# jameschapman19/cca_zoo

Hardware: NVIDIA H100
Metric: rcca_fit_per_s (higher is better)
Workload: dtype tf32x3b+f32

## Files before the change

### cca_zoo_b200/csrc/common.cuh

```cuda
#pragma once

#include <cuda.h>
#include <cuda_runtime.h>
#include <stdint.h>
#include <stdio.h>

namespace ccab {

void set_error(const char* fmt, ...);
int cuda_fail(cudaError_t e, const char* what);

#define CCAB_CUDA(expr)                                              \
  do {                                                               \
    cudaError_t _e = (expr);                                         \
    if (_e != cudaSuccess) return ::ccab::cuda_fail(_e, #expr);      \
  } while (0)

#define CCAB_CHECK_ARG(cond, ...)        \
  do {                                   \
    if (!(cond)) {                       \
      ::ccab::set_error(__VA_ARGS__);    \
      return -1;                         \
    }                                    \
  } while (0)

void count_launches(int n);
long launch_count();

static inline int64_t ceil_div(int64_t a, int64_t b) { return (a + b - 1) / b; }

#ifdef __CUDACC__

__device__ __forceinline__ uint32_t smem_u32(const void* p) {
  return static_cast<uint32_t>(__cvta_generic_to_shared(p));
}

template <int N>
__device__ __forceinline__ void setmaxnreg_dec() { asm volatile("setmaxnreg.dec.sync.aligned.u32 %0;" ::"n"(N)); }
template <int N>
__device__ __forceinline__ void setmaxnreg_inc() { asm volatile("setmaxnreg.inc.sync.aligned.u32 %0;" ::"n"(N)); }

__device__ __forceinline__ void mbar_init(uint64_t* bar, uint32_t count) {
  asm volatile("mbarrier.init.shared::cta.b64 [%0], %1;" ::"r"(smem_u32(bar)), "r"(count) : "memory");
}
__device__ __forceinline__ void fence_mbar_init() {
  asm volatile("fence.mbarrier_init.release.cluster;" ::: "memory");
}
__device__ __forceinline__ void mbar_arrive(uint64_t* bar) {
  asm volatile("mbarrier.arrive.shared::cta.b64 _, [%0];" ::"r"(smem_u32(bar)) : "memory");
}
__device__ __forceinline__ void mbar_arrive_expect_tx(uint64_t* bar, uint32_t bytes) {
  asm volatile("mbarrier.arrive.expect_tx.shared::cta.b64 _, [%0], %1;" ::"r"(smem_u32(bar)), "r"(bytes)
               : "memory");
}
__device__ __forceinline__ bool mbar_try_wait(uint64_t* bar, uint32_t parity) {
  uint32_t ok;
  asm volatile(
      "{\n\t.reg .pred P1;\n\t"
      "mbarrier.try_wait.parity.shared::cta.b64 P1, [%1], %2;\n\t"
      "selp.b32 %0, 1, 0, P1;\n\t}\n"
      : "=r"(ok)
      : "r"(smem_u32(bar)), "r"(parity)
      : "memory");
  return ok != 0;
}
__device__ __forceinline__ void mbar_wait(uint64_t* bar, uint32_t parity) {
  uint32_t spins = 0;
  while (!mbar_try_wait(bar, parity)) {
    if (++spins > (1u << 25)) __trap();
  }
}

__device__ __forceinline__ void tma_load_2d(void* smem_dst, const CUtensorMap* map, uint64_t* bar, int c0, int c1) {
  asm volatile(
      "cp.async.bulk.tensor.2d.shared::cluster.global.mbarrier::complete_tx::bytes [%0], [%1, {%3, %4}], [%2];"
      ::"r"(smem_u32(smem_dst)), "l"(map), "r"(smem_u32(bar)), "r"(c0), "r"(c1)
      : "memory");
}


__device__ __forceinline__ void fence_proxy_async_smem() {
  asm volatile("fence.proxy.async.shared::cta;" ::: "memory");
}
__device__ __forceinline__ void wgmma_fence() { asm volatile("wgmma.fence.sync.aligned;" ::: "memory"); }
__device__ __forceinline__ void wgmma_commit() { asm volatile("wgmma.commit_group.sync.aligned;" ::: "memory"); }
__device__ __forceinline__ void wgmma_wait_all() { asm volatile("wgmma.wait_group.sync.aligned 0;" ::: "memory"); }
__device__ __forceinline__ void wgmma_wait_1() { asm volatile("wgmma.wait_group.sync.aligned 1;" ::: "memory"); }
template <int R>
__device__ __forceinline__ void wgmma_fence_regs(float* d) {
#pragma unroll
  for (int i = 0; i < R; ++i) asm volatile("" : "+f"(d[i])::"memory");
}

__device__ __forceinline__ uint64_t wgmma_desc_k128(uint32_t saddr) {
  return (uint64_t)((saddr >> 4) & 0x3FFF) | ((uint64_t)1 << 16) | ((uint64_t)(1024 >> 4) << 32) |
         ((uint64_t)1 << 62);
}

template <int N>
__device__ __forceinline__ void wgmma_tf32(float* d, uint64_t desc_a, uint64_t desc_b);

template <>
__device__ __forceinline__ void wgmma_tf32<64>(float* d, uint64_t desc_a, uint64_t desc_b) {
  asm volatile(
      "{\n\t.reg .pred p;\n\tsetp.ne.b32 p, %34, 0;\n\t"
      "wgmma.mma_async.sync.aligned.m64n64k8.f32.tf32.tf32 "
      "{%0, %1, %2, %3, %4, %5, %6, %7, %8, %9, %10, %11, %12, %13, %14, %15, %16, %17, %18, %19, %20, %21, %22, %23, %24, %25, %26, %27, %28, %29, %30, %31}, %32, %33, p, 1, 1;\n\t}\n"
      : "+f"(d[0]), "+f"(d[1]), "+f"(d[2]), "+f"(d[3]), "+f"(d[4]), "+f"(d[5]), "+f"(d[6]), "+f"(d[7]), "+f"(d[8]), "+f"(d[9]), "+f"(d[10]), "+f"(d[11]), "+f"(d[12]), "+f"(d[13]), "+f"(d[14]), "+f"(d[15]), "+f"(d[16]), "+f"(d[17]), "+f"(d[18]), "+f"(d[19]), "+f"(d[20]), "+f"(d[21]), "+f"(d[22]), "+f"(d[23]), "+f"(d[24]), "+f"(d[25]), "+f"(d[26]), "+f"(d[27]), "+f"(d[28]), "+f"(d[29]), "+f"(d[30]), "+f"(d[31])
      : "l"(desc_a), "l"(desc_b), "r"(1));
}

template <>
__device__ __forceinline__ void wgmma_tf32<128>(float* d, uint64_t desc_a, uint64_t desc_b) {
  asm volatile(
      "{\n\t.reg .pred p;\n\tsetp.ne.b32 p, %66, 0;\n\t"
      "wgmma.mma_async.sync.aligned.m64n128k8.f32.tf32.tf32 "
      "{%0, %1, %2, %3, %4, %5, %6, %7, %8, %9, %10, %11, %12, %13, %14, %15, %16, %17, %18, %19, %20, %21, %22, %23, %24, %25, %26, %27, %28, %29, %30, %31, %32, %33, %34, %35, %36, %37, %38, %39, %40, %41, %42, %43, %44, %45, %46, %47, %48, %49, %50, %51, %52, %53, %54, %55, %56, %57, %58, %59, %60, %61, %62, %63}, %64, %65, p, 1, 1;\n\t}\n"
      : "+f"(d[0]), "+f"(d[1]), "+f"(d[2]), "+f"(d[3]), "+f"(d[4]), "+f"(d[5]), "+f"(d[6]), "+f"(d[7]), "+f"(d[8]), "+f"(d[9]), "+f"(d[10]), "+f"(d[11]), "+f"(d[12]), "+f"(d[13]), "+f"(d[14]), "+f"(d[15]), "+f"(d[16]), "+f"(d[17]), "+f"(d[18]), "+f"(d[19]), "+f"(d[20]), "+f"(d[21]), "+f"(d[22]), "+f"(d[23]), "+f"(d[24]), "+f"(d[25]), "+f"(d[26]), "+f"(d[27]), "+f"(d[28]), "+f"(d[29]), "+f"(d[30]), "+f"(d[31]), "+f"(d[32]), "+f"(d[33]), "+f"(d[34]), "+f"(d[35]), "+f"(d[36]), "+f"(d[37]), "+f"(d[38]), "+f"(d[39]), "+f"(d[40]), "+f"(d[41]), "+f"(d[42]), "+f"(d[43]), "+f"(d[44]), "+f"(d[45]), "+f"(d[46]), "+f"(d[47]), "+f"(d[48]), "+f"(d[49]), "+f"(d[50]), "+f"(d[51]), "+f"(d[52]), "+f"(d[53]), "+f"(d[54]), "+f"(d[55]), "+f"(d[56]), "+f"(d[57]), "+f"(d[58]), "+f"(d[59]), "+f"(d[60]), "+f"(d[61]), "+f"(d[62]), "+f"(d[63])
      : "l"(desc_a), "l"(desc_b), "r"(1));
}

__device__ __forceinline__ float tf32_hi(float v) { return __uint_as_float(__float_as_uint(v) & 0xFFFFE000u); }
__device__ __forceinline__ float tf32_residual(float v) {
  uint32_t l;
  asm("cvt.rna.tf32.f32 %0, %1;" : "=r"(l) : "f"(v - tf32_hi(v)));
  return __uint_as_float(l);
}

__device__ __forceinline__ uint32_t k128_offset(int row, int kg) {
  return (uint32_t)row * 128u + ((uint32_t)(kg ^ (row & 7)) << 4);
}

template <bool KMAJ, int ROWS>
struct TileStager {
  static constexpr int kItems = ROWS * 8 / 256;
  float v[kItems][4];

  __device__ __forceinline__ static int item_row(int i) { return KMAJ ? i >> 3 : i % ROWS; }
  __device__ __forceinline__ static int item_kg(int i) { return KMAJ ? i & 7 : i / ROWS; }

  __device__ __forceinline__ void load(const float* X, int64_t ld, int rows, int ks, bool vec) {
#pragma unroll
    for (int j = 0; j < kItems; ++j) {
      const int i = threadIdx.x + 256 * j;
      const int r = item_row(i), k = 4 * item_kg(i);
      if (KMAJ) {
        const float* src = X + (int64_t)r * ld + k;
        if (vec && r < rows && k + 4 <= ks) {
          const float4 q = __ldg(reinterpret_cast<const float4*>(src));
          v[j][0] = q.x; v[j][1] = q.y; v[j][2] = q.z; v[j][3] = q.w;
        } else {
#pragma unroll
          for (int e = 0; e < 4; ++e) v[j][e] = (r < rows && k + e < ks) ? __ldg(src + e) : 0.f;
        }
      } else {
#pragma unroll
        for (int e = 0; e < 4; ++e) v[j][e] = (r < rows && k + e < ks) ? __ldg(X + (int64_t)(k + e) * ld + r) : 0.f;
      }
    }
  }

  template <bool X3>
  __device__ __forceinline__ void store(uint8_t* hi, uint8_t* lo) const {
#pragma unroll
    for (int j = 0; j < kItems; ++j) {
      const int i = threadIdx.x + 256 * j;
      const uint32_t off = k128_offset(item_row(i), item_kg(i));
      *reinterpret_cast<float4*>(hi + off) =
          make_float4(tf32_hi(v[j][0]), tf32_hi(v[j][1]), tf32_hi(v[j][2]), tf32_hi(v[j][3]));
      if (X3)
        *reinterpret_cast<float4*>(lo + off) = make_float4(tf32_residual(v[j][0]), tf32_residual(v[j][1]),
                                                           tf32_residual(v[j][2]), tf32_residual(v[j][3]));
    }
  }
};

#endif

}
```

### cca_zoo_b200/csrc/moments.cu

```cuda
#include "moments.cuh"

#include <mutex>
#include <type_traits>

namespace ccab {

int make_layout(int n_views, const int64_t* dims, ColumnLayout* L) {
  CCAB_CHECK_ARG(n_views >= 1 && n_views <= kMaxViews, "n_views must be in [1,%d], got %d", kMaxViews,
                 n_views);
  L->n_views = n_views;
  L->coff[0] = 0;
  L->poff[0] = 0;
  int nb = 0;
  for (int v = 0; v < n_views; ++v) {
    CCAB_CHECK_ARG(dims[v] >= 1 && dims[v] <= kMaxBlocks * kBlk, "bad view width %lld", (long long)dims[v]);
    L->dims[v] = (int)dims[v];
    int b = (int)ceil_div(dims[v], kBlk);
    nb += b;
    L->coff[v + 1] = L->coff[v] + (int)dims[v];
    L->poff[v + 1] = L->poff[v] + b * kBlk;
  }
  CCAB_CHECK_ARG(nb <= kMaxBlocks, "total padded width %d exceeds %d", nb * kBlk, kMaxBlocks * kBlk);
  L->nblocks = nb;
  L->D = L->coff[n_views];
  L->Dp = nb * kBlk;
  return 0;
}

static bool g_prof_on = false;
static cudaEvent_t g_prof_e0 = nullptr, g_prof_e1 = nullptr;
static bool g_prof_valid = false;
void moments_profile_enable(int on) {
  g_prof_on = on != 0;
  g_prof_valid = false;
  if (g_prof_on && !g_prof_e0) {
    cudaEventCreate(&g_prof_e0);
    cudaEventCreate(&g_prof_e1);
  }
}
float moments_profile_last_ms() {
  if (!g_prof_valid) return -1.f;
  float ms = -1.f;
  if (cudaEventSynchronize(g_prof_e1) != cudaSuccess) return -1.f;
  if (cudaEventElapsedTime(&ms, g_prof_e0, g_prof_e1) != cudaSuccess) return -1.f;
  return ms;
}

struct WgParams {
  CUtensorMap map[kMaxViews];
  uint8_t blk_view[kMaxBlocks];
  int blk_col0[kMaxBlocks];
  float* partial;
  float* partial_sum;
  int64_t n_rows, rows_per_split;
  int64_t row_base;
  int nblocks, Dp;
};
static_assert(sizeof(WgParams) <= 4096, "kernel parameter space");

constexpr int kWgXpose = 256;
constexpr int kWgThreads = kWgXpose + 256;
constexpr int kWgKC = 32;
constexpr int kWgTile = kBlk * kWgKC * 4;

template <bool X3>
struct WgCfg {
  static constexpr int kOps = X3 ? 2 : 1;
  static constexpr int kOpStage = 2 * kOps * kWgTile;
  static constexpr int kRawStage = 2 * kWgTile;
  static constexpr int kOpStages = X3 ? 2 : 3;
  static constexpr int kRawStages = X3 ? 3 : 4;
  static constexpr int kBarOff = kOpStages * kOpStage + kRawStages * kRawStage;
  static constexpr int kSumOff = kBarOff + 2 * (kOpStages + kRawStages) * 8;
  static constexpr int kSmem = kSumOff + kBlk * 4 + 1024;
};
static_assert(WgCfg<true>::kSmem <= 227 * 1024 && WgCfg<false>::kSmem <= 227 * 1024, "shared memory per block");

template <bool X3>
__global__ void __launch_bounds__(kWgThreads, 1) moments_wgmma_kernel(const __grid_constant__ WgParams p) {
  using Cfg = WgCfg<X3>;
  constexpr int NO = Cfg::kOpStages, NR = Cfg::kRawStages;
  extern __shared__ uint8_t smem_raw[];
  uint8_t* smem = smem_raw + ((1024u - (smem_u32(smem_raw) & 1023u)) & 1023u);
  uint8_t* ops = smem;
  uint8_t* raw = smem + NO * Cfg::kOpStage;
  uint64_t* raw_full = reinterpret_cast<uint64_t*>(smem + Cfg::kBarOff);
  uint64_t* raw_empty = raw_full + NR;
  uint64_t* op_full = raw_empty + NR;
  uint64_t* op_empty = op_full + NO;

  int t = blockIdx.x, bi = 0, rowlen = p.nblocks;
  while (t >= rowlen) { t -= rowlen; ++bi; --rowlen; }
  const int bj = bi + t;
  const bool diag = bi == bj;
  const int split = blockIdx.y;
  const int64_t r0 = (int64_t)split * p.rows_per_split;
  const int64_t r1 = min(r0 + p.rows_per_split, p.n_rows);
  const int nch = r1 > r0 ? (int)((r1 - r0 + kWgKC - 1) / kWgKC) : 0;

  if (threadIdx.x == 0) {
    for (int s = 0; s < NR; ++s) {
      mbar_init(&raw_full[s], 1);
      mbar_init(&raw_empty[s], kWgXpose);
    }
    for (int s = 0; s < NO; ++s) {
      mbar_init(&op_full[s], kWgXpose);
      mbar_init(&op_empty[s], 8);
    }
    fence_mbar_init();
  }
  __syncthreads();

  if (threadIdx.x < kWgXpose) {
    setmaxnreg_dec<80>();
    const int m = threadIdx.x % kBlk, h = threadIdx.x / kBlk;
    const CUtensorMap* mapA = &p.map[p.blk_view[bi]];
    const CUtensorMap* mapB = &p.map[p.blk_view[bj]];
    const int colA = p.blk_col0[bi], colB = p.blk_col0[bj];
    auto issue = [&](int c) {
      const int s = c % NR;
      const int row = (int)(p.row_base + r0 + (int64_t)c * kWgKC);
      mbar_arrive_expect_tx(&raw_full[s], diag ? kWgTile : 2 * kWgTile);
      tma_load_2d(raw + s * Cfg::kRawStage, mapA, &raw_full[s], colA, row);
      if (!diag) tma_load_2d(raw + s * Cfg::kRawStage + kWgTile, mapB, &raw_full[s], colB, row);
    };
    if (threadIdx.x == 0)
      for (int c = 0; c < min(NR, nch); ++c) issue(c);

    float csum = 0.f;
    auto transpose = [&](const float* src, uint8_t* hi, uint8_t* lo, bool sums) {
#pragma unroll
      for (int j = 0; j < kWgKC / 8; ++j) {
        const int kg = 2 * j + h;
        float v[4];
#pragma unroll
        for (int e = 0; e < 4; ++e) v[e] = src[(4 * kg + e) * kBlk + m];
        const uint32_t off = k128_offset(m, kg);
        *reinterpret_cast<float4*>(hi + off) = make_float4(tf32_hi(v[0]), tf32_hi(v[1]), tf32_hi(v[2]), tf32_hi(v[3]));
        if (X3)
          *reinterpret_cast<float4*>(lo + off) = make_float4(tf32_residual(v[0]), tf32_residual(v[1]),
                                                             tf32_residual(v[2]), tf32_residual(v[3]));
        if (sums) csum += (v[0] + v[1]) + (v[2] + v[3]);
      }
    };
    for (int c = 0; c < nch; ++c) {
      const int sr = c % NR, so = c % NO;
      mbar_wait(&raw_full[sr], (c / NR) & 1);
      mbar_wait(&op_empty[so], ((c / NO) & 1) ^ 1);
      const float* src = reinterpret_cast<const float*>(raw + sr * Cfg::kRawStage);
      uint8_t* dst = ops + so * Cfg::kOpStage;
      transpose(src, dst, dst + kWgTile, diag);
      if (!diag) transpose(src + kBlk * kWgKC, dst + Cfg::kOps * kWgTile, dst + (Cfg::kOps + 1) * kWgTile, false);
      fence_proxy_async_smem();
      mbar_arrive(&raw_empty[sr]);
      mbar_arrive(&op_full[so]);
      if (threadIdx.x == 0 && c + NR < nch) {
        mbar_wait(&raw_empty[sr], (c / NR) & 1);
        issue(c + NR);
      }
    }
    if (diag) {
      float* odd = reinterpret_cast<float*>(smem + Cfg::kSumOff);
      if (h) odd[m] = csum;
      asm volatile("bar.sync 1, %0;" ::"n"(kWgXpose) : "memory");
      if (!h) p.partial_sum[(size_t)split * p.Dp + bi * kBlk + m] = csum + odd[m];
    }
  } else {
    setmaxnreg_inc<168>();
    const int wg = (threadIdx.x - kWgXpose) >> 7;
    float acc[64];
#pragma unroll
    for (int i = 0; i < 64; ++i) acc[i] = 0.f;
    wgmma_fence_regs<64>(acc);
    for (int c = 0; c < nch; ++c) {
      const int so = c % NO;
      mbar_wait(&op_full[so], (c / NO) & 1);
      const uint32_t st = smem_u32(ops + so * Cfg::kOpStage);
      const uint32_t a0 = st + wg * 64 * 128;
      const uint32_t b0 = diag ? st : st + Cfg::kOps * kWgTile;
      wgmma_fence();
#pragma unroll
      for (int kk = 0; kk < kWgKC / 8; ++kk) {
        const uint64_t a_hi = wgmma_desc_k128(a0 + 32 * kk), b_hi = wgmma_desc_k128(b0 + 32 * kk);
        if (X3) {
          const uint64_t a_lo = wgmma_desc_k128(a0 + kWgTile + 32 * kk), b_lo = wgmma_desc_k128(b0 + kWgTile + 32 * kk);
          wgmma_tf32<128>(acc, a_lo, b_hi);
          wgmma_tf32<128>(acc, a_hi, b_lo);
        }
        wgmma_tf32<128>(acc, a_hi, b_hi);
      }
      wgmma_commit();
      wgmma_wait_1();
      if (c > 0 && (threadIdx.x & 31) == 0) mbar_arrive(&op_empty[(c - 1) % NO]);
    }
    wgmma_wait_all();
    wgmma_fence_regs<64>(acc);

    const int warp = (threadIdx.x >> 5) & 3, lane = threadIdx.x & 31;
    float* P = p.partial + (size_t)split * p.Dp * p.Dp;
    const int row0 = bi * kBlk + wg * 64 + warp * 16 + (lane >> 2);
    const int col0 = bj * kBlk + 2 * (lane & 3);
#pragma unroll
    for (int r = 0; r < 64; r += 2) {
      const int row = row0 + 8 * ((r >> 1) & 1), col = col0 + 8 * (r >> 2);
      *reinterpret_cast<float2*>(P + (size_t)row * p.Dp + col) = make_float2(acc[r], acc[r + 1]);
    }
  }
}
struct SimtParams {
  const void* view_ptr[kMaxViews];
  int64_t view_ld[kMaxViews];
  int view_dim[kMaxViews];
  int view_poff[kMaxViews + 1];
  int n_views;
  int64_t n_rows;
  int64_t rows_per_split;
  int nb64, Dp;
  void* partial;
  void* partial_sum;
};

template <typename T>
__global__ void __launch_bounds__(256) moments_simt_kernel(const SimtParams p) {
  constexpr int KC = 16;
  __shared__ T As[KC][64];
  __shared__ T Bs[KC][64];
  int t = blockIdx.x, bi = 0, rowlen = p.nb64;
  while (t >= rowlen) { t -= rowlen; ++bi; --rowlen; }
  const int bj = bi + t;
  const int split = blockIdx.y;
  const int64_t r0 = split * p.rows_per_split;
  const int64_t r1 = min(r0 + p.rows_per_split, p.n_rows);

  auto locate = [&](int pcol0, int& v, int& c0) {
    v = 0;
    while (v + 1 < p.n_views && p.view_poff[v + 1] <= pcol0) ++v;
    c0 = pcol0 - p.view_poff[v];
  };
  int vA, cA, vB, cB;
  locate(bi * 64, vA, cA);
  locate(bj * 64, vB, cB);
  const T* XA = static_cast<const T*>(p.view_ptr[vA]);
  const T* XB = static_cast<const T*>(p.view_ptr[vB]);
  const int64_t ldA = p.view_ld[vA], ldB = p.view_ld[vB];
  const int dA = p.view_dim[vA], dB = p.view_dim[vB];

  const int tx = threadIdx.x & 15, ty = threadIdx.x >> 4;
  T acc[4][4];
#pragma unroll
  for (int i = 0; i < 4; ++i)
#pragma unroll
    for (int j = 0; j < 4; ++j) acc[i][j] = T(0);
  T csum[4] = {T(0), T(0), T(0), T(0)};

  const int lc = threadIdx.x & 63, lr = threadIdx.x >> 6;
  for (int64_t r = r0; r < r1; r += KC) {
#pragma unroll
    for (int i = 0; i < KC / 4; ++i) {
      const int kr = lr + 4 * i;
      const int64_t row = r + kr;
      const bool rv = row < r1;
      As[kr][lc] = (rv && cA + lc < dA) ? XA[row * ldA + cA + lc] : T(0);
      Bs[kr][lc] = (rv && cB + lc < dB) ? XB[row * ldB + cB + lc] : T(0);
    }
    __syncthreads();
#pragma unroll
    for (int k = 0; k < KC; ++k) {
      T a[4], b[4];
#pragma unroll
      for (int i = 0; i < 4; ++i) { a[i] = As[k][ty * 4 + i]; b[i] = Bs[k][tx * 4 + i]; }
#pragma unroll
      for (int i = 0; i < 4; ++i)
#pragma unroll
        for (int j = 0; j < 4; ++j) acc[i][j] = fma(a[i], b[j], acc[i][j]);
      if (ty == 0) {
#pragma unroll
        for (int j = 0; j < 4; ++j) csum[j] += b[j];
      }
    }
    __syncthreads();
  }
  T* P = static_cast<T*>(p.partial) + (size_t)split * p.Dp * p.Dp;
#pragma unroll
  for (int i = 0; i < 4; ++i)
#pragma unroll
    for (int j = 0; j < 4; ++j)
      P[(size_t)(bi * 64 + ty * 4 + i) * p.Dp + bj * 64 + tx * 4 + j] = acc[i][j];
  if (bi == bj && ty == 0) {
    T* S = static_cast<T*>(p.partial_sum) + (size_t)split * p.Dp;
#pragma unroll
    for (int j = 0; j < 4; ++j) S[bi * 64 + tx * 4 + j] = csum[j];
  }
}

__device__ __forceinline__ void dmma_m8n8k4(double& c0, double& c1, double a, double b) {
  asm volatile("mma.sync.aligned.m8n8k4.row.col.f64.f64.f64.f64 {%0, %1}, {%2}, {%3}, {%0, %1};"
               : "+d"(c0), "+d"(c1)
               : "d"(a), "d"(b));
}

__global__ void __launch_bounds__(256) moments_dmma_kernel(const SimtParams p) {
  constexpr int KC = 16;
  constexpr int LDS = 64 + 4;
  __shared__ double As[2][KC][LDS];
  __shared__ double Bs[2][KC][LDS];
  int t = blockIdx.x, bi = 0, rowlen = p.nb64;
  while (t >= rowlen) { t -= rowlen; ++bi; --rowlen; }
  const int bj = bi + t;
  const int split = blockIdx.y;
  const int64_t r0 = split * p.rows_per_split;
  const int64_t r1 = min(r0 + p.rows_per_split, p.n_rows);

  auto locate = [&](int pcol0, int& v, int& c0) {
    v = 0;
    while (v + 1 < p.n_views && p.view_poff[v + 1] <= pcol0) ++v;
    c0 = pcol0 - p.view_poff[v];
  };
  int vA, cA, vB, cB;
  locate(bi * 64, vA, cA);
  locate(bj * 64, vB, cB);
  const double* XA = static_cast<const double*>(p.view_ptr[vA]);
  const double* XB = static_cast<const double*>(p.view_ptr[vB]);
  const int64_t ldA = p.view_ld[vA], ldB = p.view_ld[vB];
  const int dA = p.view_dim[vA], dB = p.view_dim[vB];

  const int warp = threadIdx.x >> 5, lane = threadIdx.x & 31;
  const int wm = (warp & 1) * 32, wn = (warp >> 1) * 16;
  const int gq = lane >> 2, tq = lane & 3;
  double acc[4][2][2];
#pragma unroll
  for (int i = 0; i < 4; ++i)
#pragma unroll
    for (int j = 0; j < 2; ++j) acc[i][j][0] = acc[i][j][1] = 0.0;
  double csum = 0.0;

  const int lc = threadIdx.x & 63, lr = threadIdx.x >> 6;
  double ra[KC / 4], rb[KC / 4];
  auto gload = [&](int64_t r) {
#pragma unroll
    for (int i = 0; i < KC / 4; ++i) {
      const int64_t row = r + lr + 4 * i;
      const bool rv = row < r1;
      ra[i] = (rv && cA + lc < dA) ? XA[row * ldA + cA + lc] : 0.0;
      rb[i] = (rv && cB + lc < dB) ? XB[row * ldB + cB + lc] : 0.0;
    }
  };
  auto sstore = [&](int buf) {
#pragma unroll
    for (int i = 0; i < KC / 4; ++i) {
      As[buf][lr + 4 * i][lc] = ra[i];
      Bs[buf][lr + 4 * i][lc] = rb[i];
    }
  };
  gload(r0);
  sstore(0);
  __syncthreads();
  int buf = 0;
  for (int64_t r = r0; r < r1; r += KC, buf ^= 1) {
    const bool more = r + KC < r1;
    if (more) gload(r + KC);
#pragma unroll
    for (int k0 = 0; k0 < KC; k0 += 4) {
      double a[4], b[2];
#pragma unroll
      for (int i = 0; i < 4; ++i) a[i] = As[buf][k0 + tq][wm + 8 * i + gq];
#pragma unroll
      for (int j = 0; j < 2; ++j) b[j] = Bs[buf][k0 + tq][wn + 8 * j + gq];
#pragma unroll
      for (int i = 0; i < 4; ++i)
#pragma unroll
        for (int j = 0; j < 2; ++j) dmma_m8n8k4(acc[i][j][0], acc[i][j][1], a[i], b[j]);
    }
    if (bi == bj && threadIdx.x < 64) {
#pragma unroll
      for (int k = 0; k < KC; ++k) csum += Bs[buf][k][threadIdx.x];
    }
    if (more) sstore(buf ^ 1);
    __syncthreads();
  }
  double* P = static_cast<double*>(p.partial) + (size_t)split * p.Dp * p.Dp;
#pragma unroll
  for (int i = 0; i < 4; ++i)
#pragma unroll
    for (int j = 0; j < 2; ++j) {
      const int row = bi * 64 + wm + 8 * i + gq;
      const int col = bj * 64 + wn + 8 * j + 2 * tq;
      *reinterpret_cast<double2*>(P + (size_t)row * p.Dp + col) = make_double2(acc[i][j][0], acc[i][j][1]);
    }
  if (bi == bj && threadIdx.x < 64)
    static_cast<double*>(p.partial_sum)[(size_t)split * p.Dp + bi * 64 + threadIdx.x] = csum;
}

template <typename T>
__global__ void reduce_partials_kernel(const T* __restrict__ partial, const T* __restrict__ partial_sum,
                                       int S, int Dp, int ldp, int blk, double* __restrict__ out,
                                       int accumulate = 0) {
  const size_t total = (size_t)Dp * Dp + (partial_sum ? Dp : 0);
  const size_t slab = (size_t)ldp * ldp;
  for (size_t i = blockIdx.x * (size_t)blockDim.x + threadIdx.x; i < total;
       i += (size_t)gridDim.x * blockDim.x) {
    double acc = 0.0;
    if (i < (size_t)Dp * Dp) {
      const int r = (int)(i / Dp), c = (int)(i % Dp);
      if (r / blk <= c / blk) {
        const T* src = partial + (size_t)r * ldp + c;
        int s = 0;
        for (; s + 8 <= S; s += 8) {
          T v[8];
#pragma unroll
          for (int u = 0; u < 8; ++u) v[u] = src[(size_t)(s + u) * slab];
#pragma unroll
          for (int u = 0; u < 8; ++u) acc += (double)v[u];
        }
        for (; s < S; ++s) acc += (double)src[(size_t)s * slab];
      }
    } else {
      const size_t j = i - (size_t)Dp * Dp;
      for (int s = 0; s < S; ++s) acc += (double)partial_sum[(size_t)s * ldp + j];
    }
    out[i] = accumulate ? out[i] + acc : acc;
  }
}

struct CovParams {
  int n_views, D, Dp;
  int dims[kMaxViews];
  int coff[kMaxViews + 1];
  int poff[kMaxViews + 1];
};

__device__ __forceinline__ int compact_to_padded(const CovParams& p, int g) {
  int v = 0;
  while (v + 1 < p.n_views && p.coff[v + 1] <= g) ++v;
  return p.poff[v] + (g - p.coff[v]);
}

template <typename Tout>
__global__ void covariance_kernel(const CovParams p, const double* __restrict__ mom, double n_total,
                                  int center, Tout* __restrict__ C, int64_t ldc, Tout* __restrict__ mean) {
  const double* M = mom;
  const double* s = mom + (size_t)p.Dp * p.Dp;
  const int gi = blockIdx.y * blockDim.y + threadIdx.y;
  const int gj = blockIdx.x * blockDim.x + threadIdx.x;
  if (gi >= p.D || gj >= p.D) return;
  const int pi = compact_to_padded(p, gi), pj = compact_to_padded(p, gj);
  const int r = min(pi, pj), c = max(pi, pj);
  double v = M[(size_t)r * p.Dp + c];
  if (center) v -= s[pi] * s[pj] / n_total;
  C[(size_t)gi * ldc + gj] = (Tout)(v / (n_total - 1.0));
  if (gi == 0 && mean) mean[gj] = (Tout)(center ? s[pj] / n_total : 0.0);
}

namespace {

int sm_count() {
  static int n[64] = {};
  int dev = 0;
  cudaGetDevice(&dev);
  if (dev < 0 || dev >= 64) return 132;
  if (!n[dev]) {
    cudaDeviceGetAttribute(&n[dev], cudaDevAttrMultiProcessorCount, dev);
    if (n[dev] <= 0) n[dev] = 132;
  }
  return n[dev];
}

struct TcPlan {
  int total_chunks, num_splits, chunks_per_split, ntiles;
  size_t partial_bytes, sum_bytes;
};

TcPlan plan_tc(const ColumnLayout& L, int64_t n_rows, int mode) {
  const bool x3 = mode != 0;
  TcPlan P;
  P.total_chunks = (int)ceil_div(n_rows, kWgKC);
  P.ntiles = L.nblocks * (L.nblocks + 1) / 2;
  int S = (int)ceil_div(4 * sm_count(), P.ntiles);
  int max_splits = 64;
  if (x3) {
    S = std::max<int64_t>(S, ceil_div(n_rows, 2048));
    max_splits = 256;
  }
  const int min_chunks = 8;
  S = (int)std::min<int64_t>(S, std::max<int64_t>(1, P.total_chunks / min_chunks));
  const int64_t slab = (int64_t)L.Dp * L.Dp * (int64_t)sizeof(float);
  max_splits = (int)std::max<int64_t>(1, std::min<int64_t>(max_splits, ((int64_t)2 << 30) / slab));
  S = std::min(S, max_splits);
  S = std::max(1, std::min(S, P.total_chunks));
  P.chunks_per_split = (int)ceil_div(P.total_chunks, S);
  P.num_splits = (int)ceil_div(P.total_chunks, P.chunks_per_split);
  P.partial_bytes = (size_t)P.num_splits * L.Dp * L.Dp * sizeof(float);
  P.sum_bytes = (size_t)P.num_splits * L.Dp * sizeof(float);
  return P;
}

int64_t tc_rows_cap(const ColumnLayout& L, int mode) {
  if (mode == 0) return (int64_t)1 << 31;
  const int64_t slab = (int64_t)L.Dp * L.Dp * (int64_t)sizeof(float);
  const int64_t max_splits = std::max<int64_t>(1, std::min<int64_t>(256, ((int64_t)2 << 30) / slab));
  return max_splits * 2048;
}

inline size_t align256(size_t x) { return (x + 255) & ~size_t(255); }

struct SimtPlan {
  int nb64, ntiles, num_splits;
  int64_t rows_per_split;
};

SimtPlan plan_simt(const ColumnLayout& L, int64_t n_rows) {
  SimtPlan P;
  P.nb64 = L.Dp / 64;
  P.ntiles = P.nb64 * (P.nb64 + 1) / 2;
  int S = 1;
  if (P.ntiles < 2 * sm_count()) S = (2 * sm_count()) / P.ntiles;
  S = (int)std::min<int64_t>(S, std::max<int64_t>(1, n_rows / 64));
  S = std::max(1, std::min(S, 64));
  P.rows_per_split = ceil_div(ceil_div(n_rows, S), 16) * 16;
  P.num_splits = (int)ceil_div(n_rows, P.rows_per_split);
  return P;
}

}

size_t moments_workspace_bytes(int dtype, int precision, const ColumnLayout& L, int64_t n_rows) {
  if (precision == 2 || dtype == 1) {
    SimtPlan P = plan_simt(L, n_rows);
    size_t el = dtype == 1 ? 8 : 4;
    return align256((size_t)P.num_splits * L.Dp * L.Dp * el) + align256((size_t)P.num_splits * L.Dp * el);
  }
  TcPlan P = plan_tc(L, std::min(n_rows, tc_rows_cap(L, precision)), precision);
  return align256(P.partial_bytes) + align256(P.sum_bytes) + 256;
}

namespace {

typedef CUresult (*EncodeTiledFn)(CUtensorMap*, CUtensorMapDataType, cuuint32_t, void*, const cuuint64_t*,
                                  const cuuint64_t*, const cuuint32_t*, const cuuint32_t*, CUtensorMapInterleave,
                                  CUtensorMapSwizzle, CUtensorMapL2promotion, CUtensorMapFloatOOBfill);

EncodeTiledFn encode_fn() {
  static EncodeTiledFn fn = nullptr;
  static std::once_flag once;
  std::call_once(once, [] {
    void* f = nullptr;
    cudaDriverEntryPointQueryResult q;
    if (cudaGetDriverEntryPoint("cuTensorMapEncodeTiled", &f, cudaEnableDefault, &q) == cudaSuccess &&
        q == cudaDriverEntryPointSuccess)
      fn = reinterpret_cast<EncodeTiledFn>(f);
  });
  return fn;
}

int encode_view_map(CUtensorMap* map, const void* ptr, int64_t n_rows, int64_t d, int64_t ld) {
  EncodeTiledFn enc = encode_fn();
  if (!enc) {
    set_error("cuTensorMapEncodeTiled entry point not available (driver too old?)");
    return -2;
  }
  cuuint64_t gdim[2] = {(cuuint64_t)d, (cuuint64_t)n_rows};
  cuuint64_t gstride[1] = {(cuuint64_t)ld * 4};
  cuuint32_t box[2] = {(cuuint32_t)kBlk, (cuuint32_t)kWgKC};
  cuuint32_t estr[2] = {1, 1};
  CUresult r = enc(map, CU_TENSOR_MAP_DATA_TYPE_FLOAT32, 2, const_cast<void*>(ptr), gdim, gstride, box, estr,
                   CU_TENSOR_MAP_INTERLEAVE_NONE, CU_TENSOR_MAP_SWIZZLE_NONE, CU_TENSOR_MAP_L2_PROMOTION_L2_256B,
                   CU_TENSOR_MAP_FLOAT_OOB_FILL_NONE);
  if (r != CUDA_SUCCESS) {
    set_error("cuTensorMapEncodeTiled failed with CUresult %d (d=%lld n=%lld ld=%lld)", (int)r, (long long)d,
              (long long)n_rows, (long long)ld);
    return -3;
  }
  return 0;
}

int moments_tf32_pass(const ColumnLayout& L, WgParams& prm, int64_t row_base, int64_t n_rows, int mode,
                      double* moments_out, void* ws, size_t ws_bytes, cudaStream_t stream, int accumulate);

}

int moments_tf32(const ColumnLayout& L, const void* const* views, const int64_t* lds, int64_t n_rows, int mode,
                 double* moments_out, void* ws, size_t ws_bytes, cudaStream_t stream) {
  CCAB_CHECK_ARG(n_rows >= 1 && n_rows < (int64_t)1 << 31, "n_rows out of range");
  for (int v = 0; v < L.n_views; ++v)
    CCAB_CHECK_ARG((reinterpret_cast<uintptr_t>(views[v]) & 15) == 0 && lds[v] % 4 == 0,
                   "TF32 moments need 16-byte aligned views and lds %% 4 == 0 (view %d: ld %lld)", v,
                   (long long)lds[v]);
  {
    int dev = 0;
    CCAB_CUDA(cudaGetDevice(&dev));
    CCAB_CUDA(cudaSetDevice(dev));
  }
  WgParams prm;
  memset(&prm, 0, sizeof(prm));
  for (int v = 0; v < L.n_views; ++v) {
    int rc = encode_view_map(&prm.map[v], views[v], n_rows, L.dims[v], lds[v]);
    if (rc) return rc;
  }
  int b = 0;
  for (int v = 0; v < L.n_views; ++v)
    for (int c = 0; c < L.dims[v]; c += kBlk, ++b) {
      prm.blk_view[b] = (uint8_t)v;
      prm.blk_col0[b] = c;
    }
  const int64_t cap = tc_rows_cap(L, mode);
  if (n_rows <= cap) return moments_tf32_pass(L, prm, 0, n_rows, mode, moments_out, ws, ws_bytes, stream, 0);
  const int64_t npass = ceil_div(n_rows, cap);
  const int64_t per = std::min(cap, ceil_div(ceil_div(n_rows, npass), 2048) * 2048);
  int pass = 0;
  for (int64_t r0 = 0; r0 < n_rows; r0 += per, ++pass) {
    int rc = moments_tf32_pass(L, prm, r0, std::min(per, n_rows - r0), mode, moments_out, ws, ws_bytes, stream,
                               pass > 0);
    if (rc) return rc;
  }
  return 0;
}

namespace {
int moments_tf32_pass(const ColumnLayout& L, WgParams& prm, int64_t row_base, int64_t n_rows, int mode,
                      double* moments_out, void* ws, size_t ws_bytes, cudaStream_t stream, int accumulate) {
  TcPlan P = plan_tc(L, n_rows, mode);
  const size_t need = align256(P.partial_bytes) + align256(P.sum_bytes) + 256;
  CCAB_CHECK_ARG(ws_bytes >= need, "workspace too small: %zu < %zu", ws_bytes, need);
  uint8_t* w = reinterpret_cast<uint8_t*>((reinterpret_cast<uintptr_t>(ws) + 255) & ~uintptr_t(255));
  float* d_partial = reinterpret_cast<float*>(w);
  float* d_partial_sum = reinterpret_cast<float*>(w + align256(P.partial_bytes));

  prm.partial = d_partial;
  prm.partial_sum = d_partial_sum;
  prm.n_rows = n_rows;
  prm.rows_per_split = (int64_t)P.chunks_per_split * kWgKC;
  prm.row_base = row_base;
  prm.nblocks = L.nblocks;
  prm.Dp = L.Dp;
  dim3 grid(P.ntiles, P.num_splits);
  if (g_prof_on) cudaEventRecord(g_prof_e0, stream);
  if (mode != 0) {
    CCAB_CUDA(cudaFuncSetAttribute(moments_wgmma_kernel<true>, cudaFuncAttributeMaxDynamicSharedMemorySize,
                                   WgCfg<true>::kSmem));
    moments_wgmma_kernel<true><<<grid, kWgThreads, WgCfg<true>::kSmem, stream>>>(prm);
  } else {
    CCAB_CUDA(cudaFuncSetAttribute(moments_wgmma_kernel<false>, cudaFuncAttributeMaxDynamicSharedMemorySize,
                                   WgCfg<false>::kSmem));
    moments_wgmma_kernel<false><<<grid, kWgThreads, WgCfg<false>::kSmem, stream>>>(prm);
  }
  count_launches(1);
  CCAB_CUDA(cudaGetLastError());
  if (g_prof_on) {
    cudaEventRecord(g_prof_e1, stream);
    g_prof_valid = true;
  }

  const size_t total = (size_t)L.Dp * L.Dp + L.Dp;
  int rblocks = (int)std::min<size_t>((total + 255) / 256, (size_t)sm_count() * 8);
  reduce_partials_kernel<float><<<rblocks, 256, 0, stream>>>(d_partial, d_partial_sum, P.num_splits, L.Dp, L.Dp,
                                                            kBlk, moments_out, accumulate); count_launches(1);
  CCAB_CUDA(cudaGetLastError());
  return 0;
}
}

template <typename T>
int moments_simt(const ColumnLayout& L, const void* const* views, const int64_t* lds, int64_t n_rows,
                 double* moments_out, void* ws, size_t ws_bytes, cudaStream_t stream) {
  CCAB_CHECK_ARG(n_rows >= 1, "n_rows must be positive");
  SimtPlan P = plan_simt(L, n_rows);
  const size_t pb = align256((size_t)P.num_splits * L.Dp * L.Dp * sizeof(T));
  const size_t sb = align256((size_t)P.num_splits * L.Dp * sizeof(T));
  CCAB_CHECK_ARG(ws_bytes >= pb + sb, "workspace too small: %zu < %zu", ws_bytes, pb + sb);
  uint8_t* w = static_cast<uint8_t*>(ws);
  SimtParams prm;
  memset(&prm, 0, sizeof(prm));
  for (int v = 0; v < L.n_views; ++v) {
    prm.view_ptr[v] = views[v];
    prm.view_ld[v] = lds[v];
    prm.view_dim[v] = L.dims[v];
  }
  for (int v = 0; v <= L.n_views; ++v) prm.view_poff[v] = L.poff[v];
  prm.n_views = L.n_views;
  prm.n_rows = n_rows;
  prm.rows_per_split = P.rows_per_split;
  prm.nb64 = P.nb64;
  prm.Dp = L.Dp;
  prm.partial = w;
  prm.partial_sum = w + pb;
  dim3 grid(P.ntiles, P.num_splits);
  if constexpr (std::is_same<T, double>::value)
    moments_dmma_kernel<<<grid, 256, 0, stream>>>(prm);
  else
    moments_simt_kernel<T><<<grid, 256, 0, stream>>>(prm);
  count_launches(1);
  CCAB_CUDA(cudaGetLastError());
  const size_t total = (size_t)L.Dp * L.Dp + L.Dp;
  int rblocks = (int)std::min<size_t>((total + 255) / 256, (size_t)sm_count() * 8);
  reduce_partials_kernel<T><<<rblocks, 256, 0, stream>>>(static_cast<const T*>(prm.partial),
                                                        static_cast<const T*>(prm.partial_sum), P.num_splits,
                                                        L.Dp, L.Dp, 64, moments_out); count_launches(1);
  CCAB_CUDA(cudaGetLastError());
  return 0;
}

template int moments_simt<float>(const ColumnLayout&, const void* const*, const int64_t*, int64_t, double*, void*,
                                 size_t, cudaStream_t);
template int moments_simt<double>(const ColumnLayout&, const void* const*, const int64_t*, int64_t, double*, void*,
                                  size_t, cudaStream_t);

__global__ void pack_moments_kernel(const double* __restrict__ mom, int nblocks, int Dp, double n_local,
                                    double* __restrict__ packed) {
  const int nt = nblocks * (nblocks + 1) / 2;
  const int t = blockIdx.x;
  if (t < nt) {
    int bi = 0, rem = t, rowlen = nblocks;
    while (rem >= rowlen) { rem -= rowlen; ++bi; --rowlen; }
    const int bj = bi + rem;
    const double* src = mom + (size_t)bi * kBlk * Dp + (size_t)bj * kBlk;
    double* dst = packed + (size_t)t * kBlk * kBlk;
    for (int e = threadIdx.x; e < kBlk * kBlk; e += blockDim.x) dst[e] = src[(size_t)(e / kBlk) * Dp + (e % kBlk)];
  } else {
    double* dst = packed + (size_t)nt * kBlk * kBlk;
    const double* s = mom + (size_t)Dp * Dp;
    for (int e = threadIdx.x; e < Dp; e += blockDim.x) dst[e] = s[e];
    if (threadIdx.x == 0) { dst[Dp] = n_local; dst[Dp + 1] = 0.0; }
  }
}

__global__ void unpack_moments_kernel(const double* __restrict__ packed, int nblocks, int Dp, double* __restrict__ mom) {
  const int nt = nblocks * (nblocks + 1) / 2;
  const int bi = blockIdx.y, bj = blockIdx.x;
  if (bi < nblocks) {
    double* dst = mom + (size_t)bi * kBlk * Dp + (size_t)bj * kBlk;
    if (bj >= bi) {
      const int t = bi * nblocks - bi * (bi - 1) / 2 + (bj - bi);
      const double* src = packed + (size_t)t * kBlk * kBlk;
      for (int e = threadIdx.x; e < kBlk * kBlk; e += blockDim.x) dst[(size_t)(e / kBlk) * Dp + (e % kBlk)] = src[e];
    } else {
      for (int e = threadIdx.x; e < kBlk * kBlk; e += blockDim.x) dst[(size_t)(e / kBlk) * Dp + (e % kBlk)] = 0.0;
    }
  } else if (bj == 0) {
    const double* src = packed + (size_t)nt * kBlk * kBlk;
    double* s = mom + (size_t)Dp * Dp;
    for (int e = threadIdx.x; e < Dp; e += blockDim.x) s[e] = src[e];
  }
}

__device__ __forceinline__ double multimem_ld_reduce_add_f64(const double* mc_addr) {
  double v;
  asm volatile("multimem.ld_reduce.relaxed.sys.global.add.f64 %0, [%1];" : "=d"(v) : "l"(mc_addr) : "memory");
  return v;
}
__device__ __forceinline__ void multimem_st_f64(double* mc_addr, double v) {
  asm volatile("multimem.st.relaxed.sys.global.f64 [%0], %1;" ::"l"(mc_addr), "d"(v) : "memory");
}
__device__ __forceinline__ void st_release_sys_u32(uint32_t* p, uint32_t v) {
  asm volatile("st.release.sys.global.u32 [%0], %1;" ::"l"(p), "r"(v) : "memory");
}
__device__ __forceinline__ uint32_t ld_acquire_sys_u32(const uint32_t* p) {
  uint32_t v;
  asm volatile("ld.acquire.sys.global.u32 %0, [%1];" : "=r"(v) : "l"(p) : "memory");
  return v;
}

struct ExchangeParams {
  double* mom;
  double* sym;
  double* mc;
  uint32_t* const* pads;
  double* n_total_out;
  double n_local;
  long long packed;
  long long chunk;
  int rank, world, nblocks, Dp;
  unsigned epoch;
};

__device__ __forceinline__ const double* packed_src(const ExchangeParams& p, long long e, int nt) {
  const long long blk = e / (kBlk * kBlk);
  if (blk < nt) {
    int bi = 0, rem = (int)blk, rowlen = p.nblocks;
    while (rem >= rowlen) { rem -= rowlen; ++bi; --rowlen; }
    const int bj = bi + rem;
    const int off = (int)(e - blk * (kBlk * kBlk));
    return p.mom + ((size_t)bi * kBlk + off / kBlk) * p.Dp + (size_t)bj * kBlk + (off % kBlk);
  }
  const long long t = e - (long long)nt * kBlk * kBlk;
  return t < p.Dp ? p.mom + (size_t)p.Dp * p.Dp + t : nullptr;
}

__device__ __forceinline__ void exchange_barrier(const ExchangeParams& p, unsigned value) {
  __threadfence_system();
  __syncthreads();
  if ((int)threadIdx.x < p.world)
    st_release_sys_u32(p.pads[threadIdx.x] + (size_t)blockIdx.x * p.world + p.rank, value);
  if ((int)threadIdx.x < p.world) {
    const uint32_t* slot = p.pads[p.rank] + (size_t)blockIdx.x * p.world + threadIdx.x;
    unsigned spins = 0;
    while ((int)(ld_acquire_sys_u32(slot) - value) < 0) {
      if (++spins > (1u << 26)) {
        printf("ccab: exchange barrier timed out (rank %d cta %d peer %d)\n", p.rank, blockIdx.x, threadIdx.x);
        __trap();
      }
    }
  }
  __syncthreads();
}

__global__ void __launch_bounds__(512) exchange_nvls_kernel(const ExchangeParams p) {
  const int nt = p.nblocks * (p.nblocks + 1) / 2;
  const long long sub = (p.chunk + gridDim.x - 1) / gridDim.x;
  const long long r0 = (long long)blockIdx.x * sub;
  const long long r1 = r0 + sub < p.chunk ? r0 + sub : p.chunk;
  for (int rho = 0; rho < p.world; ++rho) {
    const long long base = (long long)rho * p.chunk;
    for (long long i = r0 + threadIdx.x; i < r1; i += blockDim.x) {
      const long long e = base + i;
      double v = 0.0;
      if (e < p.packed) {
        const double* src = packed_src(p, e, nt);
        v = src ? *src : (e == (long long)nt * kBlk * kBlk + p.Dp ? p.n_local : 0.0);
      }
      p.sym[e] = v;
    }
  }
  exchange_barrier(p, p.epoch);
  {
    const long long base = (long long)p.rank * p.chunk;
    for (long long i = r0 + threadIdx.x; i < r1; i += blockDim.x) {
      const double v = multimem_ld_reduce_add_f64(p.mc + base + i);
      multimem_st_f64(p.mc + base + i, v);
    }
  }
  exchange_barrier(p, p.epoch + 1);
  for (int rho = 0; rho < p.world; ++rho) {
    const long long base = (long long)rho * p.chunk;
    for (long long i = r0 + threadIdx.x; i < r1; i += blockDim.x) {
      const long long e = base + i;
      if (e >= p.packed) continue;
      const double v = p.sym[e];
      const double* dst = packed_src(p, e, nt);
      if (dst) *const_cast<double*>(dst) = v;
      else if (e == (long long)nt * kBlk * kBlk + p.Dp && p.n_total_out) *p.n_total_out = v;
    }
  }
}

int moments_exchange_nvls(const ColumnLayout& L, double* mom, double n_local, double* sym_local, double* sym_multicast,
                          void* const* pads_dev, int rank, int world, int pad_slots, int64_t sym_doubles,
                          unsigned epoch, double* n_total_out, cudaStream_t stream) {
  CCAB_CHECK_ARG(world >= 2 && world <= 64 && rank >= 0 && rank < world, "bad rank / world %d / %d", rank, world);
  CCAB_CHECK_ARG(mom && sym_local && sym_multicast && pads_dev, "null pointer argument");
  ExchangeParams p;
  memset(&p, 0, sizeof(p));
  p.mom = mom; p.sym = sym_local; p.mc = sym_multicast;
  p.pads = reinterpret_cast<uint32_t* const*>(pads_dev);
  p.n_total_out = n_total_out; p.n_local = n_local;
  p.packed = moments_packed_size(L);
  p.chunk = ceil_div(ceil_div(p.packed, world), 2) * 2;
  CCAB_CHECK_ARG(sym_doubles >= p.chunk * world, "symmetric buffer too small: %lld < %lld doubles", (long long)sym_doubles,
                 (long long)(p.chunk * world));
  p.rank = rank; p.world = world; p.nblocks = L.nblocks; p.Dp = L.Dp; p.epoch = epoch;
  int grid = std::min(64, pad_slots / world);
  CCAB_CHECK_ARG(grid >= 1, "signal pad too small for %d ranks", world);
  grid = (int)std::min<int64_t>(grid, std::max<int64_t>(1, p.chunk / 512));
  exchange_nvls_kernel<<<grid, 512, 0, stream>>>(p);
  count_launches(1);
  CCAB_CUDA(cudaGetLastError());
  return 0;
}

template <typename T>
// ... 157 lines not shown
```

Measured before the change: 115.6.

## Feed wgmma A operand from registers loaded directly from swizzled raw TMA tiles

The MMA warpgroups now read the A-side tile straight from the raw TMA stage into registers, split it into tf32 hi/lo parts there, and issue register-A wgmma. The transpose warps only produce the B-side operand tile, which halves the op stage size. TMA loads switch to 32-column boxes with 128B swizzle so the register reads avoid bank conflicts. Raw stages go up to five, and the refill schedule and barrier counts change so the MMA warps also release raw stages. In exchange, the MMA warps do more scalar work, use more registers, and the barrier protocol becomes more intricate.

```diff
diff --git a/cca_zoo_b200/csrc/common.cuh b/cca_zoo_b200/csrc/common.cuh
--- a/cca_zoo_b200/csrc/common.cuh
+++ b/cca_zoo_b200/csrc/common.cuh
@@ -86,10 +86,17 @@
 __device__ __forceinline__ void wgmma_commit() { asm volatile("wgmma.commit_group.sync.aligned;" ::: "memory"); }
 __device__ __forceinline__ void wgmma_wait_all() { asm volatile("wgmma.wait_group.sync.aligned 0;" ::: "memory"); }
 __device__ __forceinline__ void wgmma_wait_1() { asm volatile("wgmma.wait_group.sync.aligned 1;" ::: "memory"); }
+template <int N>
+__device__ __forceinline__ void wgmma_wait() { asm volatile("wgmma.wait_group.sync.aligned %0;" ::"n"(N) : "memory"); }
 template <int R>
 __device__ __forceinline__ void wgmma_fence_regs(float* d) {
 #pragma unroll
   for (int i = 0; i < R; ++i) asm volatile("" : "+f"(d[i])::"memory");
+}
+template <int R>
+__device__ __forceinline__ void wgmma_fence_regs(uint32_t* a) {
+#pragma unroll
+  for (int i = 0; i < R; ++i) asm volatile("" : "+r"(a[i])::"memory");
 }
 
 __device__ __forceinline__ uint64_t wgmma_desc_k128(uint32_t saddr) {
@@ -118,6 +125,19 @@
       "{%0, %1, %2, %3, %4, %5, %6, %7, %8, %9, %10, %11, %12, %13, %14, %15, %16, %17, %18, %19, %20, %21, %22, %23, %24, %25, %26, %27, %28, %29, %30, %31, %32, %33, %34, %35, %36, %37, %38, %39, %40, %41, %42, %43, %44, %45, %46, %47, %48, %49, %50, %51, %52, %53, %54, %55, %56, %57, %58, %59, %60, %61, %62, %63}, %64, %65, p, 1, 1;\n\t}\n"
       : "+f"(d[0]), "+f"(d[1]), "+f"(d[2]), "+f"(d[3]), "+f"(d[4]), "+f"(d[5]), "+f"(d[6]), "+f"(d[7]), "+f"(d[8]), "+f"(d[9]), "+f"(d[10]), "+f"(d[11]), "+f"(d[12]), "+f"(d[13]), "+f"(d[14]), "+f"(d[15]), "+f"(d[16]), "+f"(d[17]), "+f"(d[18]), "+f"(d[19]), "+f"(d[20]), "+f"(d[21]), "+f"(d[22]), "+f"(d[23]), "+f"(d[24]), "+f"(d[25]), "+f"(d[26]), "+f"(d[27]), "+f"(d[28]), "+f"(d[29]), "+f"(d[30]), "+f"(d[31]), "+f"(d[32]), "+f"(d[33]), "+f"(d[34]), "+f"(d[35]), "+f"(d[36]), "+f"(d[37]), "+f"(d[38]), "+f"(d[39]), "+f"(d[40]), "+f"(d[41]), "+f"(d[42]), "+f"(d[43]), "+f"(d[44]), "+f"(d[45]), "+f"(d[46]), "+f"(d[47]), "+f"(d[48]), "+f"(d[49]), "+f"(d[50]), "+f"(d[51]), "+f"(d[52]), "+f"(d[53]), "+f"(d[54]), "+f"(d[55]), "+f"(d[56]), "+f"(d[57]), "+f"(d[58]), "+f"(d[59]), "+f"(d[60]), "+f"(d[61]), "+f"(d[62]), "+f"(d[63])
       : "l"(desc_a), "l"(desc_b), "r"(1));
+}
+
+template <int N>
+__device__ __forceinline__ void wgmma_tf32_ra(float* d, const uint32_t* a, uint64_t desc_b);
+
+template <>
+__device__ __forceinline__ void wgmma_tf32_ra<128>(float* d, const uint32_t* a, uint64_t desc_b) {
+  asm volatile(
+      "{\n\t.reg .pred p;\n\tsetp.ne.b32 p, %69, 0;\n\t"
+      "wgmma.mma_async.sync.aligned.m64n128k8.f32.tf32.tf32 "
+      "{%0, %1, %2, %3, %4, %5, %6, %7, %8, %9, %10, %11, %12, %13, %14, %15, %16, %17, %18, %19, %20, %21, %22, %23, %24, %25, %26, %27, %28, %29, %30, %31, %32, %33, %34, %35, %36, %37, %38, %39, %40, %41, %42, %43, %44, %45, %46, %47, %48, %49, %50, %51, %52, %53, %54, %55, %56, %57, %58, %59, %60, %61, %62, %63}, {%64, %65, %66, %67}, %68, p, 1, 1;\n\t}\n"
+      : "+f"(d[0]), "+f"(d[1]), "+f"(d[2]), "+f"(d[3]), "+f"(d[4]), "+f"(d[5]), "+f"(d[6]), "+f"(d[7]), "+f"(d[8]), "+f"(d[9]), "+f"(d[10]), "+f"(d[11]), "+f"(d[12]), "+f"(d[13]), "+f"(d[14]), "+f"(d[15]), "+f"(d[16]), "+f"(d[17]), "+f"(d[18]), "+f"(d[19]), "+f"(d[20]), "+f"(d[21]), "+f"(d[22]), "+f"(d[23]), "+f"(d[24]), "+f"(d[25]), "+f"(d[26]), "+f"(d[27]), "+f"(d[28]), "+f"(d[29]), "+f"(d[30]), "+f"(d[31]), "+f"(d[32]), "+f"(d[33]), "+f"(d[34]), "+f"(d[35]), "+f"(d[36]), "+f"(d[37]), "+f"(d[38]), "+f"(d[39]), "+f"(d[40]), "+f"(d[41]), "+f"(d[42]), "+f"(d[43]), "+f"(d[44]), "+f"(d[45]), "+f"(d[46]), "+f"(d[47]), "+f"(d[48]), "+f"(d[49]), "+f"(d[50]), "+f"(d[51]), "+f"(d[52]), "+f"(d[53]), "+f"(d[54]), "+f"(d[55]), "+f"(d[56]), "+f"(d[57]), "+f"(d[58]), "+f"(d[59]), "+f"(d[60]), "+f"(d[61]), "+f"(d[62]), "+f"(d[63])
+      : "r"(a[0]), "r"(a[1]), "r"(a[2]), "r"(a[3]), "l"(desc_b), "r"(1));
 }
 
 __device__ __forceinline__ float tf32_hi(float v) { return __uint_as_float(__float_as_uint(v) & 0xFFFFE000u); }
diff --git a/cca_zoo_b200/csrc/moments.cu b/cca_zoo_b200/csrc/moments.cu
--- a/cca_zoo_b200/csrc/moments.cu
+++ b/cca_zoo_b200/csrc/moments.cu
@@ -62,19 +62,26 @@
 constexpr int kWgThreads = kWgXpose + 256;
 constexpr int kWgKC = 32;
 constexpr int kWgTile = kBlk * kWgKC * 4;
+constexpr int kWgBox = 32 * kWgKC * 4;
+
+__device__ __forceinline__ uint32_t raw_offset(int k, int m) {
+  return (uint32_t)(m >> 5) * kWgBox + k128_offset(k, (m & 31) >> 2) + (uint32_t)(m & 3) * 4;
+}
 
 template <bool X3>
 struct WgCfg {
   static constexpr int kOps = X3 ? 2 : 1;
-  static constexpr int kOpStage = 2 * kOps * kWgTile;
+  static constexpr int kOpStage = kOps * kWgTile;
   static constexpr int kRawStage = 2 * kWgTile;
   static constexpr int kOpStages = X3 ? 2 : 3;
-  static constexpr int kRawStages = X3 ? 3 : 4;
+  static constexpr int kRawStages = 5;
   static constexpr int kBarOff = kOpStages * kOpStage + kRawStages * kRawStage;
   static constexpr int kSumOff = kBarOff + 2 * (kOpStages + kRawStages) * 8;
   static constexpr int kSmem = kSumOff + kBlk * 4 + 1024;
 };
 static_assert(WgCfg<true>::kSmem <= 227 * 1024 && WgCfg<false>::kSmem <= 227 * 1024, "shared memory per block");
+static_assert(WgCfg<true>::kRawStages > WgCfg<true>::kOpStages && WgCfg<false>::kRawStages > WgCfg<false>::kOpStages,
+              "the refill of a raw stage must not wait on the MMA warps' current slice");
 
 template <bool X3>
 __global__ void __launch_bounds__(kWgThreads, 1) moments_wgmma_kernel(const __grid_constant__ WgParams p) {
@@ -101,7 +108,7 @@
   if (threadIdx.x == 0) {
     for (int s = 0; s < NR; ++s) {
       mbar_init(&raw_full[s], 1);
-      mbar_init(&raw_empty[s], kWgXpose);
+      mbar_init(&raw_empty[s], kWgXpose + 8);
     }
     for (int s = 0; s < NO; ++s) {
       mbar_init(&op_full[s], kWgXpose);
@@ -120,21 +127,26 @@
     auto issue = [&](int c) {
       const int s = c % NR;
       const int row = (int)(p.row_base + r0 + (int64_t)c * kWgKC);
+      uint8_t* dst = raw + s * Cfg::kRawStage;
       mbar_arrive_expect_tx(&raw_full[s], diag ? kWgTile : 2 * kWgTile);
-      tma_load_2d(raw + s * Cfg::kRawStage, mapA, &raw_full[s], colA, row);
-      if (!diag) tma_load_2d(raw + s * Cfg::kRawStage + kWgTile, mapB, &raw_full[s], colB, row);
+#pragma unroll
+      for (int q = 0; q < kBlk / 32; ++q) {
+        tma_load_2d(dst + q * kWgBox, mapA, &raw_full[s], colA + 32 * q, row);
+        if (!diag) tma_load_2d(dst + kWgTile + q * kWgBox, mapB, &raw_full[s], colB + 32 * q, row);
+      }
     };
     if (threadIdx.x == 0)
       for (int c = 0; c < min(NR, nch); ++c) issue(c);
 
     float csum = 0.f;
-    auto transpose = [&](const float* src, uint8_t* hi, uint8_t* lo, bool sums) {
+    auto transpose = [&](const uint8_t* src, uint8_t* hi, uint8_t* lo, bool sums) {
 #pragma unroll
       for (int j = 0; j < kWgKC / 8; ++j) {
         const int kg = 2 * j + h;
         float v[4];
 #pragma unroll
-        for (int e = 0; e < 4; ++e) v[e] = src[(4 * kg + e) * kBlk + m];
+        for (int e = 0; e < 4; ++e)
+          v[e] = *reinterpret_cast<const float*>(src + raw_offset(4 * kg + e, m));
         const uint32_t off = k128_offset(m, kg);
         *reinterpret_cast<float4*>(hi + off) = make_float4(tf32_hi(v[0]), tf32_hi(v[1]), tf32_hi(v[2]), tf32_hi(v[3]));
         if (X3)
@@ -147,16 +159,15 @@
       const int sr = c % NR, so = c % NO;
       mbar_wait(&raw_full[sr], (c / NR) & 1);
       mbar_wait(&op_empty[so], ((c / NO) & 1) ^ 1);
-      const float* src = reinterpret_cast<const float*>(raw + sr * Cfg::kRawStage);
       uint8_t* dst = ops + so * Cfg::kOpStage;
-      transpose(src, dst, dst + kWgTile, diag);
-      if (!diag) transpose(src + kBlk * kWgKC, dst + Cfg::kOps * kWgTile, dst + (Cfg::kOps + 1) * kWgTile, false);
+      transpose(raw + sr * Cfg::kRawStage + (diag ? 0 : kWgTile), dst, dst + kWgTile, diag);
       fence_proxy_async_smem();
       mbar_arrive(&raw_empty[sr]);
       mbar_arrive(&op_full[so]);
-      if (threadIdx.x == 0 && c + NR < nch) {
-        mbar_wait(&raw_empty[sr], (c / NR) & 1);
-        issue(c + NR);
+      const int rf = c + NR - NO + 1;
+      if (threadIdx.x == 0 && rf >= NR && rf < nch) {
+        mbar_wait(&raw_empty[rf % NR], (rf / NR - 1) & 1);
+        issue(rf);
       }
     }
     if (diag) {
@@ -167,36 +178,58 @@
     }
   } else {
     setmaxnreg_inc<168>();
-    const int wg = (threadIdx.x - kWgXpose) >> 7;
+    const int wg = (threadIdx.x - kWgXpose) >> 7, lane = threadIdx.x & 31, t = lane & 3;
+    const int m = wg * 64 + ((threadIdx.x >> 5) & 3) * 16 + (lane >> 2);
+    const int kx = t ^ ((t & 1) << 2);
+    const bool swap = t & 1;
+    const uint32_t o00 = raw_offset(kx, m), o01 = raw_offset(kx ^ 4, m);
+    const uint32_t o10 = raw_offset(kx, m + 8), o11 = raw_offset(kx ^ 4, m + 8);
     float acc[64];
 #pragma unroll
     for (int i = 0; i < 64; ++i) acc[i] = 0.f;
     wgmma_fence_regs<64>(acc);
+    constexpr int KS = kWgKC / 8;
+    uint32_t fa[KS][Cfg::kOps][4] = {};
     for (int c = 0; c < nch; ++c) {
-      const int so = c % NO;
-      mbar_wait(&op_full[so], (c / NO) & 1);
-      const uint32_t st = smem_u32(ops + so * Cfg::kOpStage);
-      const uint32_t a0 = st + wg * 64 * 128;
-      const uint32_t b0 = diag ? st : st + Cfg::kOps * kWgTile;
-      wgmma_fence();
-#pragma unroll
-      for (int kk = 0; kk < kWgKC / 8; ++kk) {
-        const uint64_t a_hi = wgmma_desc_k128(a0 + 32 * kk), b_hi = wgmma_desc_k128(b0 + 32 * kk);
-        if (X3) {
-          const uint64_t a_lo = wgmma_desc_k128(a0 + kWgTile + 32 * kk), b_lo = wgmma_desc_k128(b0 + kWgTile + 32 * kk);
-          wgmma_tf32<128>(acc, a_lo, b_hi);
-          wgmma_tf32<128>(acc, a_hi, b_lo);
+      const int sr = c % NR, so = c % NO;
+      mbar_wait(&raw_full[sr], (c / NR) & 1);
+      const uint8_t* a_src = raw + sr * Cfg::kRawStage;
+      const uint32_t b0 = smem_u32(ops + so * Cfg::kOpStage);
+#pragma unroll
+      for (int kk = 0; kk < KS; ++kk) {
+        wgmma_wait<KS - 1>();
+        wgmma_fence_regs<Cfg::kOps * 4>(&fa[kk][0][0]);
+        if (kk == KS - 1 && c > 0 && lane == 0) mbar_arrive(&op_empty[(c - 1) % NO]);
+        const uint8_t* s = a_src + kk * 1024;
+        const float v00 = *reinterpret_cast<const float*>(s + o00), v01 = *reinterpret_cast<const float*>(s + o01);
+        const float v10 = *reinterpret_cast<const float*>(s + o10), v11 = *reinterpret_cast<const float*>(s + o11);
+        const float a[4] = {swap ? v01 : v00, swap ? v11 : v10, swap ? v00 : v01, swap ? v10 : v11};
+#pragma unroll
+        for (int i = 0; i < 4; ++i) {
+          fa[kk][0][i] = __float_as_uint(tf32_hi(a[i]));
+          if constexpr (X3) fa[kk][1][i] = __float_as_uint(tf32_residual(a[i]));
         }
-        wgmma_tf32<128>(acc, a_hi, b_hi);
+        wgmma_fence_regs<Cfg::kOps * 4>(&fa[kk][0][0]);
+        if (kk == KS - 1) {
+          __syncwarp();
+          if (lane == 0) mbar_arrive(&raw_empty[sr]);
+        }
+        if (kk == 0) mbar_wait(&op_full[so], (c / NO) & 1);
+        const uint64_t b_hi = wgmma_desc_k128(b0 + 32 * kk);
+        wgmma_fence();
+        if constexpr (X3) {
+          const uint64_t b_lo = wgmma_desc_k128(b0 + kWgTile + 32 * kk);
+          wgmma_tf32_ra<128>(acc, fa[kk][1], b_hi);
+          wgmma_tf32_ra<128>(acc, fa[kk][0], b_lo);
+        }
+        wgmma_tf32_ra<128>(acc, fa[kk][0], b_hi);
+        wgmma_commit();
       }
-      wgmma_commit();
-      wgmma_wait_1();
-      if (c > 0 && (threadIdx.x & 31) == 0) mbar_arrive(&op_empty[(c - 1) % NO]);
     }
     wgmma_wait_all();
     wgmma_fence_regs<64>(acc);
 
-    const int warp = (threadIdx.x >> 5) & 3, lane = threadIdx.x & 31;
+    const int warp = (threadIdx.x >> 5) & 3;
     float* P = p.partial + (size_t)split * p.Dp * p.Dp;
     const int row0 = bi * kBlk + wg * 64 + warp * 16 + (lane >> 2);
     const int col0 = bj * kBlk + 2 * (lane & 3);
@@ -560,10 +593,10 @@
   }
   cuuint64_t gdim[2] = {(cuuint64_t)d, (cuuint64_t)n_rows};
   cuuint64_t gstride[1] = {(cuuint64_t)ld * 4};
-  cuuint32_t box[2] = {(cuuint32_t)kBlk, (cuuint32_t)kWgKC};
+  cuuint32_t box[2] = {32, (cuuint32_t)kWgKC};
   cuuint32_t estr[2] = {1, 1};
   CUresult r = enc(map, CU_TENSOR_MAP_DATA_TYPE_FLOAT32, 2, const_cast<void*>(ptr), gdim, gstride, box, estr,
-                   CU_TENSOR_MAP_INTERLEAVE_NONE, CU_TENSOR_MAP_SWIZZLE_NONE, CU_TENSOR_MAP_L2_PROMOTION_L2_256B,
+                   CU_TENSOR_MAP_INTERLEAVE_NONE, CU_TENSOR_MAP_SWIZZLE_128B, CU_TENSOR_MAP_L2_PROMOTION_L2_256B,
                    CU_TENSOR_MAP_FLOAT_OOB_FILL_NONE);
   if (r != CUDA_SUCCESS) {
     set_error("cuTensorMapEncodeTiled failed with CUresult %d (d=%lld n=%lld ld=%lld)", (int)r, (long long)d,
```

Measured after the change: 122.3 (median of 6 runs). 1.06x the previous value.
